# windingwind/seal-3d

Measured on AMD Instinct MI355X. Metric: train samples/s (NGP -O step on synthetic Lego 800x800 rays), higher is better.
Workload: dtype f16; 1 GPU; configs[1]: nerf_synthetic/lego-shaped NGP -O (hashgrid L16 F2 T2^19 + ffmlp 64x2/64x3 + raymarching), 800x800 cameras, 4096 rays/step/GPU; num_rays_per_gpu=4096, parallelism=ray-sharded dp1, pretrain_steps=384, launch=hip-graph replay

## Files before the change

### include/seal3d_hip.h

```cpp
#ifndef SEAL3D_HIP_H
#define SEAL3D_HIP_H

#include <stddef.h>
#include <stdint.h>

#ifdef __cplusplus
extern "C" {
#endif

typedef void* s3d_stream_t;

enum { S3D_F32 = 0, S3D_F16 = 1 };
enum { S3D_OK = 0, S3D_ERR_INVALID = 1, S3D_ERR_HIP = 2, S3D_ERR_UNSUPPORTED = 3 };

const char* s3d_last_error(void);
const char* s3d_version(void);


int s3d_near_far_from_aabb(const float* rays_o, const float* rays_d, const float* aabb, uint32_t N,
                           float min_near, float* nears, float* fars, float* noises, const int32_t* noise_step,
                           uint32_t noise_key, s3d_stream_t stream);

int s3d_sph_from_ray(const float* rays_o, const float* rays_d, float radius, uint32_t N, float* coords,
                     s3d_stream_t stream);
// ... 3 lines not shown

int s3d_morton3D(const int32_t* coords, uint32_t N, int32_t* indices, s3d_stream_t stream);

int s3d_morton3D_invert(const int32_t* indices, uint32_t N, int32_t* coords, s3d_stream_t stream);

int s3d_packbits(const float* grid, uint32_t N, float density_thresh, uint8_t* bitfield,
                 s3d_stream_t stream);

int s3d_sweep_draw(const double* u_uniform, const double* u_occupied, const int32_t* occ_csum, uint32_t N, uint32_t H,
                   float bound, float half_cell, uint32_t noise_key, const int32_t* noise_step, int32_t* cells,
                   float* xyzs, s3d_stream_t stream);
size_t s3d_sweep_update_workspace_size(uint32_t n_cells);
int s3d_sweep_update(float* density_grid, uint32_t n_cells, const int32_t* cells, const void* sigma, int sigma_dtype,
                     uint32_t n, float density_scale, float decay, void* workspace, size_t workspace_bytes,
                     float* grid_sum, int32_t* step_counter, s3d_stream_t stream);

size_t s3d_march_rays_train_workspace_size(uint32_t N, uint32_t max_steps);
int s3d_march_rays_train(const float* rays_o, const float* rays_d, const uint8_t* grid, float bound,
                         float dt_gamma, uint32_t max_steps, uint32_t N, uint32_t C, uint32_t H,
                         uint32_t M, const float* nears, const float* fars, float* xyzs, float* dirs,
                         float* deltas, int32_t* rays, int32_t* counter, const float* noises,
                         void* workspace, size_t workspace_bytes, int path, const float* aabb, float min_near,
                         const int32_t* noise_step, uint32_t noise_key, s3d_stream_t stream);

int s3d_composite_rays_train_forward(const float* sigmas, const float* rgbs, const float* deltas,
                                     const int32_t* rays, uint32_t M, uint32_t N, float T_thresh,
                                     float* weights_sum, float* depth, float* image, int path,
                                     s3d_stream_t stream);

int s3d_composite_rays_train_backward(const float* grad_weights_sum, const float* grad_image,
// ... 290 lines not shown
```

### seal-3d_amd/csrc/raymarching.hip

```cpp
#include "s3d_common.hpp"

namespace s3d {
namespace {

constexpr float kSqrt3 = 1.7320508075688772f;
constexpr float kRPi = 0.3183098861837907f;

__device__ __forceinline__ uint32_t expand_bits_any(uint32_t v) {
    v = (v * 0x00010001u) & 0xFF0000FFu;
    v = (v * 0x00000101u) & 0x0F00F00Fu;
    v = (v * 0x00000011u) & 0xC30C30C3u;
    v = (v * 0x00000005u) & 0x49249249u;
    return v;
}
__device__ __forceinline__ uint32_t expand_bits(uint32_t v) {
    v = (v | (v << 16)) & 0xFF0000FFu;
    v = (v | (v << 8)) & 0x0F00F00Fu;
    v = (v | (v << 4)) & 0xC30C30C3u;
    v = (v | (v << 2)) & 0x49249249u;
    return v;
}
__device__ __forceinline__ uint32_t morton3d(uint32_t x, uint32_t y, uint32_t z) {
    return expand_bits(x) | (expand_bits(y) << 1) | (expand_bits(z) << 2);
}
// ... 87 lines not shown
__global__ void k_morton3d(const int32_t* __restrict__ coords, uint32_t N, int32_t* __restrict__ indices) {
    for (uint32_t n = blockIdx.x * blockDim.x + threadIdx.x; n < N; n += gridDim.x * blockDim.x)
        indices[n] = (int32_t)(expand_bits_any((uint32_t)coords[n * 3]) | (expand_bits_any((uint32_t)coords[n * 3 + 1]) << 1) |
                               (expand_bits_any((uint32_t)coords[n * 3 + 2]) << 2));
}

__global__ void k_morton3d_invert(const int32_t* __restrict__ indices, uint32_t N, int32_t* __restrict__ coords) {
    for (uint32_t n = blockIdx.x * blockDim.x + threadIdx.x; n < N; n += gridDim.x * blockDim.x) {
        const int32_t ind = indices[n];
        coords[n * 3] = (int32_t)morton3d_invert((uint32_t)(ind >> 0));
        coords[n * 3 + 1] = (int32_t)morton3d_invert((uint32_t)(ind >> 1));
        coords[n * 3 + 2] = (int32_t)morton3d_invert((uint32_t)(ind >> 2));
    }
}

__global__ void k_packbits(const float* __restrict__ grid, uint32_t N, float thresh, uint8_t* __restrict__ bitfield) {
    const float4* g4 = reinterpret_cast<const float4*>(grid);
    for (uint32_t n = blockIdx.x * blockDim.x + threadIdx.x; n < N; n += gridDim.x * blockDim.x) {
        const float4 a = g4[n * 2], b = g4[n * 2 + 1];
        uint32_t bits = 0;
        bits |= (a.x > thresh) ? 1u : 0u;   bits |= (a.y > thresh) ? 2u : 0u;
        bits |= (a.z > thresh) ? 4u : 0u;   bits |= (a.w > thresh) ? 8u : 0u;
        bits |= (b.x > thresh) ? 16u : 0u;  bits |= (b.y > thresh) ? 32u : 0u;
        bits |= (b.z > thresh) ? 64u : 0u;  bits |= (b.w > thresh) ? 128u : 0u;
        bitfield[n] = (uint8_t)bits;
    }
}

__global__ void __launch_bounds__(256) k_sweep_draw(const double* __restrict__ u_uniform, const double* __restrict__ u_occupied,
                                                    const int32_t* __restrict__ occ_csum, uint32_t N, uint32_t H, float bound,
                                                    float half_cell, uint32_t noise_key, const int32_t* __restrict__ noise_step,
                                                    int32_t* __restrict__ cells, float* __restrict__ xyzs) {
    const uint32_t i = blockIdx.x * 256 + threadIdx.x;
    if (i >= 2 * N) return;
    const uint32_t H3 = H * H * H;
    uint32_t cell;
    if (i < N) {
        const double v = u_uniform[i] * (double)H3;
        cell = v >= (double)(H3 - 1) ? H3 - 1 : (uint32_t)v;
    } else {
        const int32_t total = occ_csum[H3 - 1];
        const int32_t pick = (int32_t)(u_occupied[i - N] * (double)total);
        uint32_t lo = 0, hi = H3;
        while (lo < hi) {
            const uint32_t mid = (lo + hi) >> 1;
            if (occ_csum[mid] > pick) hi = mid; else lo = mid + 1;
        }
        cell = lo < H3 ? lo : H3 - 1;
    }
    cells[i] = (int32_t)cell;
    const uint32_t step = noise_step ? (uint32_t)*noise_step : 0u;
    const float inv = 2.0f / (float)(H - 1), span = bound - half_cell;
#pragma unroll
    for (uint32_t d = 0; d < 3; d++) {
        const float c = (float)morton3d_invert(cell >> d);
        const float r = ray_noise(noise_key, step, 3u * i + d);
        xyzs[(size_t)i * 3 + d] = __builtin_fmaf(__builtin_fmaf(2.0f, r, -1.0f), half_cell, (c * inv - 1.0f) * span);
    }
}

__global__ void __launch_bounds__(256) k_sweep_fill(float* __restrict__ tmp, uint32_t n) {
    const uint32_t i = blockIdx.x * 256 + threadIdx.x;
    if (i < n) tmp[i] = -1.0f;
}
template <typename T>
__global__ void __launch_bounds__(256) k_sweep_scatter(const int32_t* __restrict__ cells, const T* __restrict__ sigma, uint32_t n,
                                                       float scale, float* __restrict__ tmp) {
    const uint32_t i = blockIdx.x * 256 + threadIdx.x;
    if (i >= n) return;
    const float v = (float)sigma[i] * scale;
    atomicMax(reinterpret_cast<int32_t*>(tmp) + cells[i], __float_as_int(v));
}
__global__ void __launch_bounds__(256) k_sweep_update(float* __restrict__ grid, const float* __restrict__ tmp, uint32_t n, float decay,
                                                      float* __restrict__ partial) {
    __shared__ float wsum[4];
    float acc = 0.0f;
    for (uint32_t i = blockIdx.x * 256 + threadIdx.x; i < n; i += gridDim.x * 256) {
        float g = grid[i];
        const float t = tmp[i];
        if (g >= 0.0f && t >= 0.0f) { g = fmaxf(g * decay, t); grid[i] = g; }
        acc += g > 0.0f ? g : 0.0f;
    }
#pragma unroll
    for (int d = 32; d >= 1; d >>= 1) acc += __shfl_xor(acc, d, 64);
    if ((threadIdx.x & 63) == 0) wsum[threadIdx.x >> 6] = acc;
    __syncthreads();
    if (threadIdx.x == 0) partial[blockIdx.x] = (wsum[0] + wsum[1]) + (wsum[2] + wsum[3]);
}
__global__ void __launch_bounds__(256) k_sweep_mean(const float* __restrict__ partial, uint32_t nblocks, float inv_n, float* __restrict__ mean,
                                                    int32_t* __restrict__ step_counter) {
    __shared__ float wsum[4];
    float acc = 0.0f;
    for (uint32_t i = threadIdx.x; i < nblocks; i += 256) acc += partial[i];
#pragma unroll
    for (int d = 32; d >= 1; d >>= 1) acc += __shfl_xor(acc, d, 64);
    if ((threadIdx.x & 63) == 0) wsum[threadIdx.x >> 6] = acc;
    __syncthreads();
    if (threadIdx.x == 0) {
        *mean = ((wsum[0] + wsum[1]) + (wsum[2] + wsum[3])) * inv_n;
        if (step_counter) *step_counter += 1;
    }
}

struct Ray {
    float ox, oy, oz, dx, dy, dz, rdx, rdy, rdz;
};
struct MarchParams {
    float bound, dt_gamma, dt_min, dt_max, rH, H3, Cf, Hf, Hm1, halfH;
    const uint8_t* grid;
};

__device__ __forceinline__ MarchParams make_params(float bound, float dt_gamma, uint32_t max_steps, uint32_t C,
                                                   uint32_t H, const uint8_t* grid) {
    MarchParams p;
    p.bound = bound; p.dt_gamma = dt_gamma;
// ... 1374 lines not shown

S3D_EXPORT int s3d_compact_alive(const int32_t* in, uint32_t n, int32_t* out, int32_t* n_out, void* workspace,
                                 size_t workspace_bytes, const int32_t* n_in_dev, s3d_stream_t stream) {
    S3D_REQUIRE(n_out, "compact_alive: null n_out");
    if (n == 0) { S3D_HIP(hipMemsetAsync(n_out, 0, sizeof(int32_t), as_stream(stream))); return S3D_OK; }
    S3D_REQUIRE(in && out && workspace && workspace_bytes >= s3d_compact_alive_workspace_size(n),
                "compact_alive: bad arguments");
    const uint32_t nw = div_up<uint32_t>(n, 64);
    hipLaunchKernelGGL(k_compact_count, dim3(nw), dim3(64), 0, as_stream(stream), in, n, (uint32_t*)workspace, n_in_dev);
    hipLaunchKernelGGL(k_compact_write, dim3(nw), dim3(64), 0, as_stream(stream), in, n, out, n_out,
                       (const uint32_t*)workspace, n_in_dev);
    return check_launch("compact_alive");
}

constexpr uint32_t kSweepBlocks = 1024;

S3D_EXPORT int s3d_sweep_draw(const double* u_uniform, const double* u_occupied, const int32_t* occ_csum, uint32_t N, uint32_t H,
                              float bound, float half_cell, uint32_t noise_key, const int32_t* noise_step, int32_t* cells,
                              float* xyzs, s3d_stream_t stream) {
    if (N == 0) return S3D_OK;
    S3D_REQUIRE(u_uniform && u_occupied && occ_csum && cells && xyzs, "sweep_draw: null pointer");
    S3D_REQUIRE(H >= 2 && H <= 1024 && (uint64_t)2 * N < (1ull << 31), "sweep_draw: unsupported grid size H=%u or N=%u", H, N);
    hipLaunchKernelGGL(k_sweep_draw, dim3(div_up<uint32_t>(2 * N, 256)), dim3(256), 0, as_stream(stream), u_uniform, u_occupied,
                       occ_csum, N, H, bound, half_cell, noise_key, noise_step, cells, xyzs);
    return check_launch("sweep_draw");
}

S3D_EXPORT size_t s3d_sweep_update_workspace_size(uint32_t n_cells) { return ((size_t)n_cells + kSweepBlocks) * sizeof(float); }

S3D_EXPORT int s3d_sweep_update(float* density_grid, uint32_t n_cells, const int32_t* cells, const void* sigma, int sigma_dtype,
                                uint32_t n, float density_scale, float decay, void* workspace, size_t workspace_bytes,
                                float* grid_sum, int32_t* step_counter, s3d_stream_t stream) {
    S3D_REQUIRE(density_grid && n_cells > 0 && (n == 0 || (cells && sigma)) && grid_sum, "sweep_update: null pointer");
    S3D_REQUIRE(sigma_dtype == S3D_F32 || sigma_dtype == S3D_F16, "sweep_update: sigma dtype must be f32 or f16");
    S3D_REQUIRE(workspace && workspace_bytes >= s3d_sweep_update_workspace_size(n_cells), "sweep_update: workspace too small");
    hipStream_t st = as_stream(stream);
    float* tmp = (float*)workspace;
    float* partial = tmp + n_cells;
    hipLaunchKernelGGL(k_sweep_fill, dim3(div_up<uint32_t>(n_cells, 256)), dim3(256), 0, st, tmp, n_cells);
    if (n) {
        if (sigma_dtype == S3D_F16)
            hipLaunchKernelGGL(k_sweep_scatter<_Float16>, dim3(div_up<uint32_t>(n, 256)), dim3(256), 0, st, cells, (const _Float16*)sigma, n,
                               density_scale, tmp);
        else
            hipLaunchKernelGGL(k_sweep_scatter<float>, dim3(div_up<uint32_t>(n, 256)), dim3(256), 0, st, cells, (const float*)sigma, n,
                               density_scale, tmp);
    }
    const uint32_t blocks = std::min<uint32_t>(kSweepBlocks, div_up<uint32_t>(n_cells, 256));
    hipLaunchKernelGGL(k_sweep_update, dim3(blocks), dim3(256), 0, st, density_grid, (const float*)tmp, n_cells, decay, partial);
    hipLaunchKernelGGL(k_sweep_mean, dim3(1), dim3(256), 0, st, (const float*)partial, blocks, 1.0f, grid_sum, step_counter);
    return check_launch("sweep_update");
}
```

### seal-3d_amd/nerf/renderer.py

```python
import math

import numpy as np
import torch
import torch.nn as nn

import raymarching
import s3d_hip


import contextlib

_null_context = contextlib.nullcontext


def _meshgrid(*args):
    return torch.meshgrid(*args, indexing="ij")


def sample_pdf(bins, weights, n_samples, det=False):
    weights = weights + 1e-5
    pdf = weights / torch.sum(weights, -1, keepdim=True)
    cdf = torch.cumsum(pdf, -1)
    cdf = torch.cat([torch.zeros_like(cdf[..., :1]), cdf], -1)
    if det:
# ... 3 lines not shown
        u = torch.rand(list(cdf.shape[:-1]) + [n_samples]).to(weights.device)
    u = u.contiguous()
    inds = torch.searchsorted(cdf, u, right=True)
    below = torch.clamp(inds - 1, min=0)
    above = torch.clamp(inds, max=cdf.shape[-1] - 1)
    pick = torch.stack([below, above], -1)
    shape = [pick.shape[0], pick.shape[1], cdf.shape[-1]]
    cdf_g = torch.gather(cdf.unsqueeze(1).expand(shape), 2, pick)
    bins_g = torch.gather(bins.unsqueeze(1).expand(shape), 2, pick)
    denom = cdf_g[..., 1] - cdf_g[..., 0]
    denom = torch.where(denom < 1e-5, torch.ones_like(denom), denom)
    t = (u - cdf_g[..., 0]) / denom
    return bins_g[..., 0] + t * (bins_g[..., 1] - bins_g[..., 0])


class NeRFRenderer(nn.Module):
    def __init__(self, bound=1, cuda_ray=False, density_scale=1, min_near=0.2, density_thresh=0.01, bg_radius=-1,
                 device_compaction=True, infer_batch_scale=1):
        super().__init__()
        self.bound = bound
        self.cascade = 1 + math.ceil(math.log2(bound))
        self.grid_size = 128
        self.density_scale = density_scale
        self.min_near = min_near
        self.density_thresh = density_thresh
        self.bg_radius = bg_radius
        self.device_compaction = device_compaction
        self.sync_every = 4
        self.infer_batch_scale = infer_batch_scale

        aabb = torch.FloatTensor([-bound, -bound, -bound, bound, bound, bound])
# ... 299 lines not shown

    @torch.no_grad()
    def _pick_occupied(self, cas, N):
        grid = self.density_grid[cas]
        csum = torch.cumsum(grid > 0, dim=0, dtype=torch.int32)
        pick = (self._sorted_uniform(N, grid.device) * csum[-1]).to(torch.int32)
        return torch.searchsorted(csum, pick, right=True).clamp_(max=grid.shape[0] - 1)

    @torch.no_grad()
    def partial_grid_update_device(self, decay=0.95):
        dev = self.density_grid.device
        H3 = self.grid_size ** 3
        N = H3 // 4
        if dev.type == "cuda" and self.density_grid.dtype == torch.float32:
            R = s3d_hip.RaymarchingBackend
            if getattr(self, "_sweep_step", None) is None or self._sweep_step.device != dev:
                self._sweep_step = torch.zeros(1, dtype=torch.int32, device=dev)
                self._sweep_key = torch.initial_seed() & 0xFFFFFFFF
            total = None
            for cas in range(self.cascade):
                bound, hgs = self._cascade_geometry(cas)
                grid = self.density_grid[cas]
                csum = torch.cumsum(grid > 0, dim=0, dtype=torch.int32)
                cells, xyzs = R.sweep_draw(self._sorted_uniform(N, dev), self._sorted_uniform(N, dev), csum, self.grid_size, bound,
                                           hgs, self._sweep_key + cas, self._sweep_step)
                sigma = self.density(xyzs)["sigma"].reshape(-1).detach()
                if sigma.dtype not in (torch.float16, torch.float32):
                    sigma = sigma.float()
                part = R.sweep_update(grid, cells, sigma.contiguous(), self.density_scale, decay,
                                      self._sweep_step if cas == self.cascade - 1 else None)
                total = part if total is None else total + part
            return total / self.density_grid.numel()
        tmp_grid = torch.full_like(self.density_grid, -1)
        for cas in range(self.cascade):
            indices = (self._sorted_uniform(N, dev) * H3).long().clamp_(max=H3 - 1)
            coords = raymarching.morton3D_invert(indices)
            occ = self._pick_occupied(cas, N)
            occ_coords = raymarching.morton3D_invert(occ)
            indices = torch.cat([indices, occ], dim=0)
            coords = torch.cat([coords, occ_coords], dim=0)
            tmp_grid[cas, indices] = self._query_cells(coords, cas).to(tmp_grid.dtype)
        valid = (self.density_grid >= 0) & (tmp_grid >= 0)
        self.density_grid.copy_(torch.where(valid, torch.maximum(self.density_grid * decay, tmp_grid), self.density_grid))
        g = self.density_grid.clamp(min=0)
        return g.view(-1, 4096).sum(dim=1).sum() / g.numel()

    @torch.no_grad()
    def finish_extra_state(self, mean_density_dev):
        total_step = min(16, self.local_step)
        counted = self.step_counter[:max(total_step, 1), 0].sum().float()
        mean_density, count_sum = torch.stack([mean_density_dev.float().reshape(()), counted]).tolist()
        self.mean_density = mean_density
        self.iter_density += 1
        thresh = min(self.mean_density, self.density_thresh)
        self.density_bitfield = raymarching.packbits(self.density_grid, thresh, self.density_bitfield)
        if total_step > 0:
            self.mean_count = int(count_sum / total_step)
        self.local_step = 0

    def run(self, rays_o, rays_d, num_steps=128, upsample_steps=128, bg_color=None, perturb=False, **kwargs):
        prefix = rays_o.shape[:-1]
        rays_o = rays_o.contiguous().view(-1, 3)
        rays_d = rays_d.contiguous().view(-1, 3)
# ... 67 lines not shown
```

### seal-3d_amd/nerf/trainer.py

```python
import math

import torch
import torch.nn.functional as F

from gridencoder.grid import bump_weights_epoch


def psnr(pred, target):
    return -10 * math.log10(float(torch.mean((pred.float() - target.float()) ** 2)) + 1e-20)


class _BgMse(torch.autograd.Function):

    @staticmethod
    def forward(ctx, image, weights_sum, gt, bg, expected_grad=None, depth=None, gt_depth=None, depth_weight=1.0):
        import s3d_hip
        image, weights_sum, gt = image.float().contiguous(), weights_sum.float().contiguous(), gt.float().contiguous()
        loss = torch.empty((), dtype=torch.float32, device=image.device)
        ctx.pre = None
        extra = {}
        if depth is not None:
            extra = dict(depth=depth.detach().float().contiguous().reshape(-1), gt_depth=gt_depth.float().contiguous().reshape(-1),
                         depth_weight=float(depth_weight))
        if expected_grad is not None and expected_grad.dtype == torch.float32 and expected_grad.numel() == 1:
# ... 271 lines not shown
        super().__init__(model, capturable=True, **kw)
        self.capture_collectives = capture_collectives
        self.collectives_in_graph = False
        dev = next(model.parameters()).device
        self.s_ro = torch.zeros(num_rays, 3, device=dev)
        self.s_rd = torch.zeros(num_rays, 3, device=dev)
        self.s_gt = torch.zeros(num_rays, 3, device=dev)
        self.s_bg = torch.ones(num_rays, 3, device=dev)
        self.budget_factor = budget_factor
        self.graph_extra_state = graph_extra_state
        self.ues_graph, self.ues_mean, self.ues_warm = None, None, False
        self.graph = None
        self.graph_opt = None
        self.n_captures = 0
        self.budget = 0
        self.s_loss = None
        self.s_counter = torch.zeros(2, dtype=torch.int32, device=dev)
        self.loss_ring = torch.zeros(1024, dtype=torch.float32, device=dev)
        self._pushes = 0
        self.s_cursor = torch.zeros(2, dtype=torch.int32, device=dev)
        self.noise_key = (torch.initial_seed() * 0x9E3779B1 + (self.dist.rank if self.dist is not None else 0) * 0x85EBCA6B) & 0xFFFFFFFF
        self._counter_ring = None
        self._ring_args = None
        self.s_index = torch.zeros(1, dtype=torch.int64, device=dev)
        self.s_inds_coarse = torch.zeros(1, num_rays, dtype=torch.int64, device=dev)
        self._graph_em = None
        self._graph_bg = False

    def static_batch(self):
        n = self.s_ro.shape[0]
# ... 82 lines not shown
            self.graph_opt = torch.cuda.CUDAGraph()
            with torch.cuda.graph(self.graph_opt, pool=self.graph.pool(), capture_error_mode=_CAPTURE_MODE):
                self._body_opt()
            self.collectives_in_graph = False
        model.step_counter = ring
        model._counter_prezeroed = False
        model._noise_step = None
        model.mean_count, model.local_step = saved

    def load_checkpoint(self, checkpoint, model_only=False):
        out = super().load_checkpoint(checkpoint, model_only=model_only)
        self._counter_ring = None
        self.graph = self.graph_opt = None
        return out

    def _maybe_update_extra_state(self):
        from .renderer import NeRFRenderer
        model = self.model
        if not (model.cuda_ray and self.global_step % self.update_extra_interval == 0):
            return False
        epilogue = getattr(model, "after_extra_state", None) if getattr(type(model), "extra_state_epilogue_only", False) else None
        plain = type(model).update_extra_state is NeRFRenderer.update_extra_state or epilogue is not None
        if not (self.graph_extra_state and plain and model.iter_density >= 16) or getattr(model, "dist_shard", None) is not None:
            return super()._maybe_update_extra_state()
        with torch.autocast("cuda", dtype=torch.float16, enabled=self.fp16):
            if self.ues_graph is None and not self.ues_warm:
                mean = model.partial_grid_update_device()
                self.ues_warm = True
            else:
                if self.ues_graph is None:
                    self.ues_graph = torch.cuda.CUDAGraph()
                    with torch.cuda.graph(self.ues_graph, capture_error_mode=_CAPTURE_MODE):
                        self.ues_mean = model.partial_grid_update_device()
                self.ues_graph.replay()
                mean = self.ues_mean
            model.finish_extra_state(mean)
            if epilogue is not None:
                epilogue()
        if self.dist is not None:
            self.dist.sync_extra_state(model)
        return True

    def _stage_inputs(self, rays_o, rays_d, gt_rgb, bg=None):
        dst, src = [self.s_ro, self.s_rd, self.s_gt], [rays_o, rays_d, gt_rgb]
        if bg is not None:
            dst.append(self.s_bg)
            src.append(bg)
        if all(a.data_ptr() == b.data_ptr() for a, b in zip(dst, src)):
# ... 24 lines not shown
            self._pushes += 1
        return slot

    def train_step(self, rays_o, rays_d, gt_rgb, bg_color=1, index=None, inds_coarse=None):
        self._em_batch = self._error_map_batch(index, inds_coarse, gt_rgb)
        try:
            return self._graphed_step(rays_o, rays_d, gt_rgb, bg_color)
        finally:
            self._em_batch = None

    def _graphed_step(self, rays_o, rays_d, gt_rgb, bg_color):
        model = self.model
        model.train()
        if self._maybe_update_extra_state():
            self.s_cursor[0].zero_()
            if self.graph is not None and (model.mean_count * 1.1 > self.budget or model.mean_count * 2 < self.budget):
                self.graph = None
        self.global_step += 1
        if self.graph is None and model.mean_count <= 0:
            loss = self._eager_step(rays_o, rays_d, gt_rgb, bg_color)
            self._sched_step()
            return loss
        per_ray = torch.is_tensor(bg_color)
        if per_ray:
            if type(self)._static_loss is not GraphedTrainer._static_loss:
                raise ValueError("GraphedTrainer: this trainer's captured criterion composites on bg_color=1")
            if not (bg_color.is_cuda and bg_color.dtype == torch.float32 and bg_color.numel() == self.s_bg.numel()):
                raise ValueError("GraphedTrainer: a per-ray background is an fp32 device tensor [num_rays, 3]")
            self._stage_inputs(rays_o, rays_d, gt_rgb, bg_color.detach())
        elif bg_color != 1:
            raise ValueError("GraphedTrainer: the captured step composites on the white background (bg_color=1) of the "
                             "BASELINE configs or on a per-ray background tensor; use Trainer for other background colours")
# ... 31 lines not shown
```

### seal-3d_amd/s3d_hip/__init__.py

```python
import ctypes as C
import os
import subprocess
import weakref

import torch

_HERE = os.path.dirname(os.path.abspath(__file__))
LIB_PATH = os.environ.get("S3D_HIP_LIB") or os.path.join(_HERE, "libseal3d_hip.so")
CSRC = os.path.join(os.path.dirname(_HERE), "csrc")

F32, F16 = 0, 1

EXPORTS = [
    "s3d_last_error", "s3d_version",
    "s3d_near_far_from_aabb", "s3d_sph_from_ray", "s3d_morton3D", "s3d_morton3D_invert", "s3d_mip_levels", "s3d_packbits",
    "s3d_march_rays_train_workspace_size", "s3d_march_rays_train",
    "s3d_sweep_draw", "s3d_sweep_update_workspace_size", "s3d_sweep_update",
    "s3d_composite_rays_train_forward", "s3d_composite_rays_train_backward", "s3d_composite_rays_train_loss",
    "s3d_march_rays", "s3d_composite_rays", "s3d_compact_alive_workspace_size", "s3d_compact_alive",
    "s3d_grid_level_scales", "s3d_grid_encode_forward", "s3d_grid_encode_forward_pair", "s3d_grid_corner_indices", "s3d_grid_encode_backward",
    "s3d_grid_encode_backward_workspace_size", "s3d_grid_encode_backward_control_size",
    "s3d_grad_total_variation",
    "s3d_sh_encode_forward", "s3d_sh_encode_backward", "s3d_freq_encode_forward", "s3d_freq_encode_backward", "s3d_freq_encode_pack_forward", "s3d_freq_encode_pack_backward",
    "s3d_ffmlp_forward", "s3d_ffmlp_inference", "s3d_ffmlp_ngp_pair_inference", "s3d_ffmlp_wgrad_reduce_pair", "s3d_ffmlp_backward_workspace_size", "s3d_ffmlp_backward",
    "s3d_ffmlp_fused_backward_supported",
    "s3d_ffmlp_allocate_splitk", "s3d_ffmlp_free_splitk",
    "s3d_grads_nonfinite", "s3d_adam_step", "s3d_adam_step_multi", "s3d_adam_advance", "s3d_scaler_update", "s3d_step_ring_push", "s3d_step_epilogue",
    "s3d_ngp_mid_forward", "s3d_ngp_mid_backward", "s3d_ngp_mid2_forward", "s3d_ngp_mid2_backward", "s3d_ngp_rgb_forward", "s3d_ngp_rgb_backward",
    "s3d_bg_mse_forward", "s3d_bg_mse_backward", "s3d_bg_targets", "s3d_l1_pair_workspace_size", "s3d_l1_pair_loss",
    "s3d_seal_bbox_map", "s3d_seal_map_color", "s3d_seal_map_color_image", "s3d_seal_brush_map", "s3d_seal_anchor_map", "s3d_grid_encode_backward_adam", "s3d_vm_features_forward",
    "s3d_aabb_normalize", "s3d_weighted_abs_sum_workspace_size", "s3d_weighted_abs_sum", "s3d_pack_linear_chain", "s3d_unpack_linear_chain",
    "s3d_vm_backward_max_bins", "s3d_vm_backward_keys", "s3d_vm_backward_bins_workspace_size", "s3d_vm_backward_bins",
# ... 18 lines not shown


def lib():
    global _lib
    if _lib is None:
        if not os.path.exists(LIB_PATH):
            raise RuntimeError(
                f"seal3d HIP extension not built: {LIB_PATH} is missing. Run `python -c 'import __graft_entry__ as g; "
                "g.build()'` (needs hipcc). There is no CPU fallback for the product path.")
        l = C.CDLL(LIB_PATH)
        l.s3d_last_error.restype = C.c_char_p
        l.s3d_version.restype = C.c_char_p
        for name in ("s3d_march_rays_train_workspace_size", "s3d_compact_alive_workspace_size",
                     "s3d_ffmlp_backward_workspace_size", "s3d_grid_encode_backward_workspace_size",
                     "s3d_grid_encode_backward_control_size", "s3d_l1_pair_workspace_size",
                     "s3d_sweep_update_workspace_size", "s3d_vm_backward_bins_workspace_size", "s3d_vm_backward_stage_bytes",
                     "s3d_weighted_abs_sum_workspace_size", "s3d_background_backward_workspace_size",
                     "s3d_vm_background_backward_workspace_size"):
            getattr(l, name).restype = C.c_size_t
        l.s3d_vm_backward_max_bins.restype = C.c_uint32
        l.s3d_grid_level_scales.restype = None
        _lib = l
    return _lib


def _check(rc, what):
    if rc != 0:
        msg = lib().s3d_last_error().decode("utf-8", "replace")
        raise RuntimeError(f"{what} failed (code {rc}): {msg}")


# ... 191 lines not shown

    @staticmethod
    def sweep_update(density_grid, cells, sigma, density_scale, decay, step_counter=None):
        _need(density_grid, torch.float32, "density_grid"); _need(cells, torch.int32, "cells")
        if sigma.dtype not in (torch.float16, torch.float32) or sigma.numel() != cells.numel():
            raise RuntimeError("sweep_update: sigma must be fp16 / fp32, one per cell sample")
        if step_counter is not None:
            _need(step_counter, torch.int32, "step_counter")
        n_cells = density_grid.numel()
        ws = _ws.get(lib().s3d_sweep_update_workspace_size(_u(n_cells)), density_grid.device)
        out = torch.empty((), dtype=torch.float32, device=density_grid.device)
        _check(lib().s3d_sweep_update(_p(density_grid), _u(n_cells), _p(cells), _p(sigma), C.c_int(_dt(sigma)), _u(cells.numel()),
                                      _f(density_scale), _f(decay), _p(ws), C.c_size_t(ws.numel()), _p(out), _p(step_counter),
                                      _stream()), "sweep_update")
        return out

    @staticmethod
    def sph_from_ray(rays_o, rays_d, radius, N, coords):
        _need(rays_o, torch.float32, "rays_o")
        _check(lib().s3d_sph_from_ray(_p(rays_o), _p(rays_d), _f(radius), _u(N), _p(coords), _stream()),
               "sph_from_ray")

    @staticmethod
    def morton3D(coords, N, indices):
        _need(coords, torch.int32, "coords")
        _check(lib().s3d_morton3D(_p(coords), _u(N), _p(indices), _stream()), "morton3D")

    @staticmethod
    def morton3D_invert(indices, N, coords):
        _need(indices, torch.int32, "indices")
# ... 1092 lines not shown
```

Before: 647.7 million samples/s.

## Move density-grid sweep draw, update and threshold record fully onto device kernels

Adds native GPU kernels for the occupancy-grid sweep. Occupied-cell sampling now uses per-block bit masks plus a scanned count array instead of a full cumsum, scatter and update are fused per cascade, and a tail kernel computes the mean, threshold and step count into a device record that packbits reads directly. The trainer defers the graph budget check while extra-state work is pending, so the host does not have to sync to read mean_count. This adds more kernels and a deferred budget check that may recapture graphs one step late.

```diff
diff --git a/include/seal3d_hip.h b/include/seal3d_hip.h
--- a/include/seal3d_hip.h
+++ b/include/seal3d_hip.h
@@ -41,6 +41,18 @@
 int s3d_sweep_update(float* density_grid, uint32_t n_cells, const int32_t* cells, const void* sigma, int sigma_dtype,
                      uint32_t n, float density_scale, float decay, void* workspace, size_t workspace_bytes,
                      float* grid_sum, int32_t* step_counter, s3d_stream_t stream);
+
+size_t s3d_sweep_draw_native_workspace_size(uint32_t H);
+int s3d_sweep_draw_native(const double* u_uniform, const double* u_occupied, const float* density_grid, uint32_t N, uint32_t H,
+                          float bound, float half_cell, uint32_t noise_key, const int32_t* noise_step, float* tmp, int32_t* cells,
+                          float* xyzs, void* workspace, size_t workspace_bytes, s3d_stream_t stream);
+uint32_t s3d_sweep_partial_stride(void);
+int s3d_sweep_scatter_update(float* density_grid, uint32_t n_cells, const int32_t* cells, const void* sigma, int sigma_dtype,
+                             uint32_t sigma_stride, uint32_t n, float density_scale, float decay, float* tmp, float* partial,
+                             s3d_stream_t stream);
+int s3d_sweep_tail(const float* partial, uint32_t cascades, uint32_t n_cells, float density_thresh, const int32_t* step_ring,
+                   const int32_t* local_step, int32_t* sweep_step, void* record, s3d_stream_t stream);
+int s3d_packbits_record(const float* grid, uint32_t N, const void* record, uint8_t* bitfield, s3d_stream_t stream);
 
 size_t s3d_march_rays_train_workspace_size(uint32_t N, uint32_t max_steps);
 int s3d_march_rays_train(const float* rays_o, const float* rays_d, const uint8_t* grid, float bound,
diff --git a/seal-3d_amd/csrc/raymarching.hip b/seal-3d_amd/csrc/raymarching.hip
--- a/seal-3d_amd/csrc/raymarching.hip
+++ b/seal-3d_amd/csrc/raymarching.hip
@@ -125,7 +125,7 @@
     }
 }
 
-__global__ void k_packbits(const float* __restrict__ grid, uint32_t N, float thresh, uint8_t* __restrict__ bitfield) {
+__device__ __forceinline__ void packbits_rows(const float* __restrict__ grid, uint32_t N, float thresh, uint8_t* __restrict__ bitfield) {
     const float4* g4 = reinterpret_cast<const float4*>(grid);
     for (uint32_t n = blockIdx.x * blockDim.x + threadIdx.x; n < N; n += gridDim.x * blockDim.x) {
         const float4 a = g4[n * 2], b = g4[n * 2 + 1];
@@ -137,7 +137,36 @@
         bitfield[n] = (uint8_t)bits;
     }
 }
-
+__global__ void k_packbits(const float* __restrict__ grid, uint32_t N, float thresh, uint8_t* __restrict__ bitfield) {
+    packbits_rows(grid, N, thresh, bitfield);
+}
+
+struct SweepRecord {
+    float mean;
+    float thresh;
+    uint32_t count_lo;
+    uint32_t count_hi;
+};
+__global__ void k_packbits_record(const float* __restrict__ grid, uint32_t N, const SweepRecord* __restrict__ record,
+                                  uint8_t* __restrict__ bitfield) {
+    packbits_rows(grid, N, record->thresh, bitfield);
+}
+
+__device__ __forceinline__ uint32_t sweep_uniform_cell(double u, uint32_t H3) {
+    const double v = u * (double)H3;
+    return v >= (double)(H3 - 1) ? H3 - 1 : (uint32_t)v;
+}
+__device__ __forceinline__ void sweep_emit(uint32_t i, uint32_t cell, uint32_t H, float bound, float half_cell, uint32_t noise_key,
+                                           uint32_t step, int32_t* __restrict__ cells, float* __restrict__ xyzs) {
+    cells[i] = (int32_t)cell;
+    const float inv = 2.0f / (float)(H - 1), span = bound - half_cell;
+#pragma unroll
+    for (uint32_t d = 0; d < 3; d++) {
+        const float c = (float)morton3d_invert(cell >> d);
+        const float r = ray_noise(noise_key, step, 3u * i + d);
+        xyzs[(size_t)i * 3 + d] = __builtin_fmaf(__builtin_fmaf(2.0f, r, -1.0f), half_cell, (c * inv - 1.0f) * span);
+    }
+}
 __global__ void __launch_bounds__(256) k_sweep_draw(const double* __restrict__ u_uniform, const double* __restrict__ u_occupied,
                                                     const int32_t* __restrict__ occ_csum, uint32_t N, uint32_t H, float bound,
                                                     float half_cell, uint32_t noise_key, const int32_t* __restrict__ noise_step,
@@ -147,8 +176,7 @@
     const uint32_t H3 = H * H * H;
     uint32_t cell;
     if (i < N) {
-        const double v = u_uniform[i] * (double)H3;
-        cell = v >= (double)(H3 - 1) ? H3 - 1 : (uint32_t)v;
+        cell = sweep_uniform_cell(u_uniform[i], H3);
     } else {
         const int32_t total = occ_csum[H3 - 1];
         const int32_t pick = (int32_t)(u_occupied[i - N] * (double)total);
@@ -159,14 +187,136 @@
         }
         cell = lo < H3 ? lo : H3 - 1;
     }
-    cells[i] = (int32_t)cell;
     const uint32_t step = noise_step ? (uint32_t)*noise_step : 0u;
-    const float inv = 2.0f / (float)(H - 1), span = bound - half_cell;
-#pragma unroll
-    for (uint32_t d = 0; d < 3; d++) {
-        const float c = (float)morton3d_invert(cell >> d);
-        const float r = ray_noise(noise_key, step, 3u * i + d);
-        xyzs[(size_t)i * 3 + d] = __builtin_fmaf(__builtin_fmaf(2.0f, r, -1.0f), half_cell, (c * inv - 1.0f) * span);
+    sweep_emit(i, cell, H, bound, half_cell, noise_key, step, cells, xyzs);
+}
+
+constexpr uint32_t kScanBlock = 1024;
+constexpr uint32_t kSweepCntLds = 4096;
+
+template <typename T>
+__device__ __forceinline__ T block_scan_exclusive(T mine, T* sh, T& total) {
+    const uint32_t lane = threadIdx.x & 63u, w = threadIdx.x >> 6;
+    T incl = mine;
+#pragma unroll
+    for (int d = 1; d < 64; d <<= 1) {
+        const T up = __shfl_up(incl, d, 64);
+        if (lane >= (uint32_t)d) incl = incl + up;
+    }
+    if (lane == 63u) sh[w] = incl;
+    __syncthreads();
+    const T w0 = sh[0], w1 = sh[1], w2 = sh[2], w3 = sh[3];
+    __syncthreads();
+    const T before = __shfl_up(incl, 1, 64);
+    const T lanes = lane == 0u ? T(0) : before;
+    total = ((w0 + w1) + w2) + w3;
+    const T off = w == 0 ? T(0) : (w == 1 ? w0 : (w == 2 ? w0 + w1 : (w0 + w1) + w2));
+    return off + lanes;
+}
+
+__global__ void __launch_bounds__(256) k_sweep_partials(const float* __restrict__ grid, uint32_t H3, float* __restrict__ tmp,
+                                                        int32_t* __restrict__ cnt, uint32_t* __restrict__ occ_bits, uint32_t nbc) {
+    __shared__ int32_t shi[4];
+    __shared__ uint32_t words[32];
+    const uint32_t t = threadIdx.x;
+    for (uint32_t b = blockIdx.x; b < nbc; b += gridDim.x) {
+        const uint32_t c0 = b * kScanBlock + 4u * t;
+        uint32_t nib = 0;
+#pragma unroll
+        for (uint32_t q = 0; q < 4; q++)
+            if (c0 + q < H3) {
+                nib |= grid[c0 + q] > 0.0f ? (1u << q) : 0u;
+                tmp[c0 + q] = -1.0f;
+            }
+        if (t < 32) words[t] = 0;
+        __syncthreads();
+        if (nib) atomicOr(&words[t >> 3], nib << (4u * (t & 7u)));
+        __syncthreads();
+        if (t < 32) occ_bits[b * 32u + t] = words[t];
+        int32_t total;
+        (void)block_scan_exclusive((int32_t)__popc(nib), shi, total);
+        if (t == 0) cnt[b] = total;
+    }
+}
+
+template <typename T>
+__device__ __forceinline__ void scan_inclusive_in_place(T* __restrict__ a, uint32_t n, T* sh) {
+    T carry = T(0);
+    for (uint32_t base = 0; base < n; base += kScanBlock) {
+        const uint32_t j0 = base + 4u * threadIdx.x;
+        T l[4], acc = T(0);
+#pragma unroll
+        for (uint32_t q = 0; q < 4; q++) {
+            const T v = (j0 + q < n) ? a[j0 + q] : T(0);
+            acc = q == 0 ? v : acc + v;
+            l[q] = acc;
+        }
+        T total;
+        const T pre = carry + block_scan_exclusive(acc, sh, total);
+#pragma unroll
+        for (uint32_t q = 0; q < 4; q++)
+            if (j0 + q < n) a[j0 + q] = pre + l[q];
+        carry = carry + total;
+    }
+}
+__global__ void __launch_bounds__(256) k_sweep_scan(int32_t* __restrict__ cnt, uint32_t nbc) {
+    __shared__ int32_t shi[4];
+    scan_inclusive_in_place(cnt, nbc, shi);
+}
+
+__device__ __forceinline__ uint32_t sweep_occupied_cell(int32_t pick, const int32_t* __restrict__ incl_cnt,
+                                                        const uint32_t* __restrict__ occ_bits, uint32_t nbc, uint32_t H3) {
+    uint32_t lo = 0, hi = nbc;
+    while (lo < hi) {
+        const uint32_t mid = (lo + hi) >> 1;
+        if (incl_cnt[mid] > pick) hi = mid; else lo = mid + 1;
+    }
+    if (lo >= nbc) return H3 - 1;
+    const int32_t r = pick - (lo ? incl_cnt[lo - 1] : 0);
+    const uint4* __restrict__ w4 = reinterpret_cast<const uint4*>(occ_bits + (size_t)lo * 32u);
+    uint4 v[8];
+#pragma unroll
+    for (int k = 0; k < 8; k++) v[k] = w4[k];
+    uint32_t word = 0, at = 32;
+    int32_t rest = 0, before = 0;
+#pragma unroll
+    for (int w = 0; w < 32; w++) {
+        const uint4 q = v[w >> 2];
+        const uint32_t x = (w & 3) == 0 ? q.x : ((w & 3) == 1 ? q.y : ((w & 3) == 2 ? q.z : q.w));
+        const int32_t c = (int32_t)__popc(x);
+        if (at == 32 && r < before + c) { at = (uint32_t)w; word = x; rest = r - before; }
+        before += c;
+    }
+    if (at == 32) return H3 - 1;
+    for (; rest > 0; rest--) word &= word - 1u;
+    const uint32_t cell = lo * kScanBlock + at * 32u + (uint32_t)(__ffs((int)word) - 1);
+    return cell < H3 ? cell : H3 - 1;
+}
+
+__global__ void __launch_bounds__(256) k_sweep_draw_native(const double* __restrict__ u_uniform, const double* __restrict__ u_occupied,
+                                                           const int32_t* __restrict__ incl_cnt, const uint32_t* __restrict__ occ_bits,
+                                                           uint32_t nbc, uint32_t N, uint32_t H, float bound, float half_cell,
+                                                           uint32_t noise_key, const int32_t* __restrict__ noise_step,
+                                                           int32_t* __restrict__ cells, float* __restrict__ xyzs) {
+    const uint32_t H3 = H * H * H;
+    const uint32_t step = noise_step ? (uint32_t)*noise_step : 0u;
+    __shared__ int32_t sh_cnt[kSweepCntLds];
+    const int32_t* cnt = incl_cnt;
+    if (nbc <= kSweepCntLds) {
+        for (uint32_t i = threadIdx.x; i < nbc; i += 256) sh_cnt[i] = incl_cnt[i];
+        __syncthreads();
+        cnt = sh_cnt;
+    }
+    const int32_t occupied = cnt[nbc - 1];
+    const uint32_t j0 = blockIdx.x * kScanBlock + 4u * threadIdx.x;
+#pragma unroll
+    for (uint32_t q = 0; q < 4; q++) {
+        const uint32_t j = j0 + q;
+        if (j < N) {
+            sweep_emit(j, sweep_uniform_cell(u_uniform[j], H3), H, bound, half_cell, noise_key, step, cells, xyzs);
+            const int32_t pick = (int32_t)(u_occupied[j] * (double)occupied);
+            sweep_emit(N + j, sweep_occupied_cell(pick, cnt, occ_bits, nbc, H3), H, bound, half_cell, noise_key, step, cells, xyzs);
+        }
     }
 }
 
@@ -175,11 +325,11 @@
     if (i < n) tmp[i] = -1.0f;
 }
 template <typename T>
-__global__ void __launch_bounds__(256) k_sweep_scatter(const int32_t* __restrict__ cells, const T* __restrict__ sigma, uint32_t n,
-                                                       float scale, float* __restrict__ tmp) {
+__global__ void __launch_bounds__(256) k_sweep_scatter(const int32_t* __restrict__ cells, const T* __restrict__ sigma, uint32_t stride,
+                                                       uint32_t n, float scale, float* __restrict__ tmp) {
     const uint32_t i = blockIdx.x * 256 + threadIdx.x;
     if (i >= n) return;
-    const float v = (float)sigma[i] * scale;
+    const float v = (float)sigma[(size_t)i * stride] * scale;
     atomicMax(reinterpret_cast<int32_t*>(tmp) + cells[i], __float_as_int(v));
 }
 __global__ void __launch_bounds__(256) k_sweep_update(float* __restrict__ grid, const float* __restrict__ tmp, uint32_t n, float decay,
@@ -198,18 +348,47 @@
     __syncthreads();
     if (threadIdx.x == 0) partial[blockIdx.x] = (wsum[0] + wsum[1]) + (wsum[2] + wsum[3]);
 }
+__device__ __forceinline__ float sweep_sum_partials(const float* __restrict__ partial, uint32_t nblocks, float* wsum) {
+    float acc = 0.0f;
+    for (uint32_t i = threadIdx.x; i < nblocks; i += 256) acc += partial[i];
+#pragma unroll
+    for (int d = 32; d >= 1; d >>= 1) acc += __shfl_xor(acc, d, 64);
+    if ((threadIdx.x & 63) == 0) wsum[threadIdx.x >> 6] = acc;
+    __syncthreads();
+    const float s = (wsum[0] + wsum[1]) + (wsum[2] + wsum[3]);
+    __syncthreads();
+    return s;
+}
 __global__ void __launch_bounds__(256) k_sweep_mean(const float* __restrict__ partial, uint32_t nblocks, float inv_n, float* __restrict__ mean,
                                                     int32_t* __restrict__ step_counter) {
     __shared__ float wsum[4];
-    float acc = 0.0f;
-    for (uint32_t i = threadIdx.x; i < nblocks; i += 256) acc += partial[i];
-#pragma unroll
-    for (int d = 32; d >= 1; d >>= 1) acc += __shfl_xor(acc, d, 64);
-    if ((threadIdx.x & 63) == 0) wsum[threadIdx.x >> 6] = acc;
-    __syncthreads();
+    const float s = sweep_sum_partials(partial, nblocks, wsum);
     if (threadIdx.x == 0) {
-        *mean = ((wsum[0] + wsum[1]) + (wsum[2] + wsum[3])) * inv_n;
+        *mean = s * inv_n;
         if (step_counter) *step_counter += 1;
+    }
+}
+__global__ void __launch_bounds__(256) k_sweep_tail(const float* __restrict__ partial, uint32_t cascades, uint32_t stride,
+                                                    uint32_t nblocks, float inv_n, float density_thresh,
+                                                    const int32_t* __restrict__ step_ring, const int32_t* __restrict__ local_step,
+                                                    int32_t* __restrict__ sweep_step, SweepRecord* __restrict__ record) {
+    __shared__ float wsum[4];
+    float total = 0.0f;
+    for (uint32_t c = 0; c < cascades; c++) {
+        const float s = sweep_sum_partials(partial + (size_t)c * stride, nblocks, wsum);
+        total = c == 0 ? s : total + s;
+    }
+    if (threadIdx.x == 0) {
+        const float mean = total * inv_n;
+        record->mean = mean;
+        record->thresh = density_thresh < mean ? density_thresh : mean;
+        int32_t rows = *local_step;
+        rows = rows < 0 ? 0 : (rows > 16 ? 16 : rows);
+        int64_t count = 0;
+        for (int32_t r = 0; r < rows; r++) count += step_ring[2 * r];
+        record->count_lo = (uint32_t)((uint64_t)count & 0xFFFFFFFFull);
+        record->count_hi = (uint32_t)((uint64_t)count >> 32);
+        if (sweep_step) *sweep_step += 1;
     }
 }
 
@@ -1614,6 +1793,17 @@
 }
 
 constexpr uint32_t kSweepBlocks = 1024;
+static uint32_t sweep_update_blocks(uint32_t n_cells) { return std::min<uint32_t>(kSweepBlocks, div_up<uint32_t>(n_cells, 256)); }
+static void launch_sweep_scatter(const int32_t* cells, const void* sigma, int sigma_dtype, uint32_t stride, uint32_t n, float scale,
+                                 float* tmp, hipStream_t st) {
+    if (n == 0) return;
+    if (sigma_dtype == S3D_F16)
+        hipLaunchKernelGGL(k_sweep_scatter<_Float16>, dim3(div_up<uint32_t>(n, 256)), dim3(256), 0, st, cells, (const _Float16*)sigma,
+                           stride, n, scale, tmp);
+    else
+        hipLaunchKernelGGL(k_sweep_scatter<float>, dim3(div_up<uint32_t>(n, 256)), dim3(256), 0, st, cells, (const float*)sigma, stride,
+                           n, scale, tmp);
+}
 
 S3D_EXPORT int s3d_sweep_draw(const double* u_uniform, const double* u_occupied, const int32_t* occ_csum, uint32_t N, uint32_t H,
                               float bound, float half_cell, uint32_t noise_key, const int32_t* noise_step, int32_t* cells,
@@ -1638,16 +1828,66 @@
     float* tmp = (float*)workspace;
     float* partial = tmp + n_cells;
     hipLaunchKernelGGL(k_sweep_fill, dim3(div_up<uint32_t>(n_cells, 256)), dim3(256), 0, st, tmp, n_cells);
-    if (n) {
-        if (sigma_dtype == S3D_F16)
-            hipLaunchKernelGGL(k_sweep_scatter<_Float16>, dim3(div_up<uint32_t>(n, 256)), dim3(256), 0, st, cells, (const _Float16*)sigma, n,
-                               density_scale, tmp);
-        else
-            hipLaunchKernelGGL(k_sweep_scatter<float>, dim3(div_up<uint32_t>(n, 256)), dim3(256), 0, st, cells, (const float*)sigma, n,
-                               density_scale, tmp);
-    }
-    const uint32_t blocks = std::min<uint32_t>(kSweepBlocks, div_up<uint32_t>(n_cells, 256));
+    launch_sweep_scatter(cells, sigma, sigma_dtype, 1, n, density_scale, tmp, st);
+    const uint32_t blocks = sweep_update_blocks(n_cells);
     hipLaunchKernelGGL(k_sweep_update, dim3(blocks), dim3(256), 0, st, density_grid, (const float*)tmp, n_cells, decay, partial);
     hipLaunchKernelGGL(k_sweep_mean, dim3(1), dim3(256), 0, st, (const float*)partial, blocks, 1.0f, grid_sum, step_counter);
     return check_launch("sweep_update");
 }
+
+static uint32_t sweep_cell_blocks(uint32_t H) { return div_up<uint32_t>(H * H * H, kScanBlock); }
+
+S3D_EXPORT size_t s3d_sweep_draw_native_workspace_size(uint32_t H) { return (size_t)sweep_cell_blocks(H) * 33 * sizeof(uint32_t); }
+
+S3D_EXPORT int s3d_sweep_draw_native(const double* u_uniform, const double* u_occupied, const float* density_grid, uint32_t N,
+                                     uint32_t H, float bound, float half_cell, uint32_t noise_key, const int32_t* noise_step,
+                                     float* tmp, int32_t* cells, float* xyzs, void* workspace, size_t workspace_bytes,
+                                     s3d_stream_t stream) {
+    S3D_REQUIRE(u_uniform && u_occupied && density_grid && tmp && cells && xyzs && N > 0, "sweep_draw_native: null pointer or N = 0");
+    S3D_REQUIRE(H >= 2 && H <= 1024 && (uint64_t)2 * N < (1ull << 31), "sweep_draw_native: unsupported grid size H=%u or N=%u", H, N);
+    S3D_REQUIRE(workspace && ((uintptr_t)workspace & 15) == 0 && workspace_bytes >= s3d_sweep_draw_native_workspace_size(H),
+                "sweep_draw_native: workspace too small or misaligned");
+    const uint32_t nbc = sweep_cell_blocks(H), H3 = H * H * H;
+    uint32_t* occ_bits = (uint32_t*)workspace;
+    int32_t* cnt = (int32_t*)(occ_bits + (size_t)nbc * 32);
+    hipStream_t st = as_stream(stream);
+    hipLaunchKernelGGL(k_sweep_partials, dim3(std::min<uint32_t>(nbc, 4096)), dim3(256), 0, st, density_grid, H3, tmp, cnt, occ_bits, nbc);
+    hipLaunchKernelGGL(k_sweep_scan, dim3(1), dim3(256), 0, st, cnt, nbc);
+    hipLaunchKernelGGL(k_sweep_draw_native, dim3(div_up<uint32_t>(N, kScanBlock)), dim3(256), 0, st, u_uniform, u_occupied,
+                       (const int32_t*)cnt, (const uint32_t*)occ_bits, nbc, N, H, bound, half_cell, noise_key, noise_step, cells, xyzs);
+    return check_launch("sweep_draw_native");
+}
+
+S3D_EXPORT uint32_t s3d_sweep_partial_stride(void) { return kSweepBlocks; }
+
+S3D_EXPORT int s3d_sweep_scatter_update(float* density_grid, uint32_t n_cells, const int32_t* cells, const void* sigma, int sigma_dtype,
+                                        uint32_t sigma_stride, uint32_t n, float density_scale, float decay, float* tmp,
+                                        float* partial, s3d_stream_t stream) {
+    S3D_REQUIRE(density_grid && n_cells > 0 && (n == 0 || (cells && sigma)) && tmp && partial, "sweep_scatter_update: null pointer");
+    S3D_REQUIRE(sigma_dtype == S3D_F32 || sigma_dtype == S3D_F16, "sweep_scatter_update: sigma dtype must be f32 or f16");
+    hipStream_t st = as_stream(stream);
+    launch_sweep_scatter(cells, sigma, sigma_dtype, sigma_stride, n, density_scale, tmp, st);
+    hipLaunchKernelGGL(k_sweep_update, dim3(sweep_update_blocks(n_cells)), dim3(256), 0, st, density_grid, (const float*)tmp, n_cells,
+                       decay, partial);
+    return check_launch("sweep_scatter_update");
+}
+
+S3D_EXPORT int s3d_sweep_tail(const float* partial, uint32_t cascades, uint32_t n_cells, float density_thresh,
+                              const int32_t* step_ring, const int32_t* local_step, int32_t* sweep_step, void* record,
+                              s3d_stream_t stream) {
+    S3D_REQUIRE(partial && cascades > 0 && n_cells > 0 && step_ring && local_step && record, "sweep_tail: null pointer");
+    S3D_REQUIRE(((uintptr_t)record & 3) == 0, "sweep_tail: record must be 4-byte aligned");
+    const float inv_n = 1.0f / (float)((uint64_t)cascades * n_cells);
+    hipLaunchKernelGGL(k_sweep_tail, dim3(1), dim3(256), 0, as_stream(stream), partial, cascades, kSweepBlocks,
+                       sweep_update_blocks(n_cells), inv_n, density_thresh, step_ring, local_step, sweep_step, (SweepRecord*)record);
+    return check_launch("sweep_tail");
+}
+
+S3D_EXPORT int s3d_packbits_record(const float* grid, uint32_t N, const void* record, uint8_t* bitfield, s3d_stream_t stream) {
+    if (N == 0) return S3D_OK;
+    S3D_REQUIRE(grid && bitfield && record, "packbits_record: null pointer");
+    S3D_REQUIRE(((uintptr_t)grid & 15) == 0 && ((uintptr_t)record & 3) == 0, "packbits_record: grid must be 16-byte aligned");
+    hipLaunchKernelGGL(k_packbits_record, dim3(stream_grid(N, 256)), dim3(256), 0, as_stream(stream), grid, N,
+                       (const SweepRecord*)record, bitfield);
+    return check_launch("packbits_record");
+}
diff --git a/seal-3d_amd/nerf/renderer.py b/seal-3d_amd/nerf/renderer.py
--- a/seal-3d_amd/nerf/renderer.py
+++ b/seal-3d_amd/nerf/renderer.py
@@ -41,7 +41,69 @@
     return bins_g[..., 0] + t * (bins_g[..., 1] - bins_g[..., 0])
 
 
+class _SweepState:
+
+    def __init__(self, dev):
+        self.device = dev
+        self.step = torch.zeros(1, dtype=torch.int32, device=dev)
+        self.local_step = torch.zeros(1, dtype=torch.int32, device=dev)
+        self.record = torch.zeros(4, dtype=torch.int32, device=dev)
+        self.host = torch.zeros(4, dtype=torch.int32).pin_memory()
+        self.event = torch.cuda.Event()
+        self.key = torch.initial_seed() & 0xFFFFFFFF
+        self.pending = None
+
+    def __deepcopy__(self, memo):
+        return None
+
+    def __reduce__(self):
+        return (type(None), ())
+
+
 class NeRFRenderer(nn.Module):
+    _mean_density = 0
+    _mean_count = 0
+    _sweep = None
+
+    @property
+    def mean_density(self):
+        self._resolve_extra_state()
+        return self._mean_density
+
+    @mean_density.setter
+    def mean_density(self, value):
+        self._resolve_extra_state()
+        self._mean_density = value
+
+    @property
+    def mean_count(self):
+        self._resolve_extra_state()
+        return self._mean_count
+
+    @mean_count.setter
+    def mean_count(self, value):
+        self._resolve_extra_state()
+        self._mean_count = value
+
+    def __getstate__(self):
+        self._resolve_extra_state()
+        return self.__dict__
+
+    def extra_state_pending(self):
+        return self._sweep is not None and self._sweep.pending is not None
+
+    def _resolve_extra_state(self):
+        st = self._sweep
+        if st is None or st.pending is None:
+            return
+        total_step, st.pending = st.pending, None
+        st.event.synchronize()
+        rec = st.host.numpy()
+        self._mean_density = float(rec.view(np.float32)[0])
+        if total_step > 0:
+            count = int(rec.view(np.uint32)[2]) | (int(rec.view(np.uint32)[3]) << 32)
+            self._mean_count = int(count / total_step)
+
     def __init__(self, bound=1, cuda_ray=False, density_scale=1, min_near=0.2, density_thresh=0.01, bg_radius=-1,
                  device_compaction=True, infer_batch_scale=1):
         super().__init__()
@@ -371,23 +433,25 @@
         N = H3 // 4
         if dev.type == "cuda" and self.density_grid.dtype == torch.float32:
             R = s3d_hip.RaymarchingBackend
-            if getattr(self, "_sweep_step", None) is None or self._sweep_step.device != dev:
-                self._sweep_step = torch.zeros(1, dtype=torch.int32, device=dev)
-                self._sweep_key = torch.initial_seed() & 0xFFFFFFFF
-            total = None
+            st = self._sweep
+            if st is None or st.device != dev:
+                st = self._sweep = _SweepState(dev)
+            if not torch.cuda.is_current_stream_capturing():
+                self.stage_extra_state()
+            tmp = torch.empty(H3, dtype=torch.float32, device=dev)
+            partial = torch.empty(self.cascade, R.sweep_partial_stride(), dtype=torch.float32, device=dev)
             for cas in range(self.cascade):
                 bound, hgs = self._cascade_geometry(cas)
                 grid = self.density_grid[cas]
-                csum = torch.cumsum(grid > 0, dim=0, dtype=torch.int32)
-                cells, xyzs = R.sweep_draw(self._sorted_uniform(N, dev), self._sorted_uniform(N, dev), csum, self.grid_size, bound,
-                                           hgs, self._sweep_key + cas, self._sweep_step)
+                cells, xyzs = R.sweep_draw_native(self._sorted_uniform(N, dev), self._sorted_uniform(N, dev), grid, self.grid_size,
+                                                  bound, hgs, tmp, st.key + cas, st.step)
                 sigma = self.density(xyzs)["sigma"].reshape(-1).detach()
                 if sigma.dtype not in (torch.float16, torch.float32):
                     sigma = sigma.float()
-                part = R.sweep_update(grid, cells, sigma.contiguous(), self.density_scale, decay,
-                                      self._sweep_step if cas == self.cascade - 1 else None)
-                total = part if total is None else total + part
-            return total / self.density_grid.numel()
+                R.sweep_scatter_update(grid, cells, sigma, self.density_scale, decay, tmp, partial[cas])
+            R.sweep_tail(partial, H3, self.density_thresh, self.step_counter, st.local_step, st.step, st.record)
+            R.packbits_record(self.density_grid, self.cascade * H3 // 8, st.record, self.density_bitfield)
+            return st.record
         tmp_grid = torch.full_like(self.density_grid, -1)
         for cas in range(self.cascade):
             indices = (self._sorted_uniform(N, dev) * H3).long().clamp_(max=H3 - 1)
@@ -403,7 +467,21 @@
         return g.view(-1, 4096).sum(dim=1).sum() / g.numel()
 
     @torch.no_grad()
+    def stage_extra_state(self):
+        if self._sweep is not None:
+            self._sweep.local_step.fill_(int(self.local_step))
+
+    @torch.no_grad()
     def finish_extra_state(self, mean_density_dev):
+        st = self._sweep
+        if st is not None and mean_density_dev is st.record:
+            self._resolve_extra_state()
+            st.host.copy_(st.record, non_blocking=True)
+            st.event.record()
+            st.pending = min(16, self.local_step)
+            self.iter_density += 1
+            self.local_step = 0
+            return
         total_step = min(16, self.local_step)
         counted = self.step_counter[:max(total_step, 1), 0].sum().float()
         mean_density, count_sum = torch.stack([mean_density_dev.float().reshape(()), counted]).tolist()
diff --git a/seal-3d_amd/nerf/trainer.py b/seal-3d_amd/nerf/trainer.py
--- a/seal-3d_amd/nerf/trainer.py
+++ b/seal-3d_amd/nerf/trainer.py
@@ -309,6 +309,7 @@
         self.graph_opt = None
         self.n_captures = 0
         self.budget = 0
+        self._budget_check_due = False
         self.s_loss = None
         self.s_counter = torch.zeros(2, dtype=torch.int32, device=dev)
         self.loss_ring = torch.zeros(1024, dtype=torch.float32, device=dev)
@@ -421,6 +422,11 @@
         self.graph = self.graph_opt = None
         return out
 
+    def _check_budget(self):
+        mean = self.model.mean_count
+        if self.graph is not None and (mean * 1.1 > self.budget or mean * 2 < self.budget):
+            self.graph = None
+
     def _maybe_update_extra_state(self):
         from .renderer import NeRFRenderer
         model = self.model
@@ -430,6 +436,9 @@
         plain = type(model).update_extra_state is NeRFRenderer.update_extra_state or epilogue is not None
         if not (self.graph_extra_state and plain and model.iter_density >= 16) or getattr(model, "dist_shard", None) is not None:
             return super()._maybe_update_extra_state()
+        if self._budget_check_due:
+            self._budget_check_due = False
+            self._check_budget()
         with torch.autocast("cuda", dtype=torch.float16, enabled=self.fp16):
             if self.ues_graph is None and not self.ues_warm:
                 mean = model.partial_grid_update_device()
@@ -439,6 +448,7 @@
                     self.ues_graph = torch.cuda.CUDAGraph()
                     with torch.cuda.graph(self.ues_graph, capture_error_mode=_CAPTURE_MODE):
                         self.ues_mean = model.partial_grid_update_device()
+                model.stage_extra_state()
                 self.ues_graph.replay()
                 mean = self.ues_mean
             model.finish_extra_state(mean)
@@ -493,8 +503,11 @@
         model.train()
         if self._maybe_update_extra_state():
             self.s_cursor[0].zero_()
-            if self.graph is not None and (model.mean_count * 1.1 > self.budget or model.mean_count * 2 < self.budget):
-                self.graph = None
+            pending = getattr(model, "extra_state_pending", None)
+            if pending is not None and pending():
+                self._budget_check_due = True
+            else:
+                self._check_budget()
         self.global_step += 1
         if self.graph is None and model.mean_count <= 0:
             loss = self._eager_step(rays_o, rays_d, gt_rgb, bg_color)
diff --git a/seal-3d_amd/s3d_hip/__init__.py b/seal-3d_amd/s3d_hip/__init__.py
--- a/seal-3d_amd/s3d_hip/__init__.py
+++ b/seal-3d_amd/s3d_hip/__init__.py
@@ -16,6 +16,8 @@
     "s3d_near_far_from_aabb", "s3d_sph_from_ray", "s3d_morton3D", "s3d_morton3D_invert", "s3d_mip_levels", "s3d_packbits",
     "s3d_march_rays_train_workspace_size", "s3d_march_rays_train",
     "s3d_sweep_draw", "s3d_sweep_update_workspace_size", "s3d_sweep_update",
+    "s3d_sweep_draw_native_workspace_size", "s3d_sweep_draw_native", "s3d_sweep_partial_stride", "s3d_sweep_scatter_update",
+    "s3d_sweep_tail", "s3d_packbits_record",
     "s3d_composite_rays_train_forward", "s3d_composite_rays_train_backward", "s3d_composite_rays_train_loss",
     "s3d_march_rays", "s3d_composite_rays", "s3d_compact_alive_workspace_size", "s3d_compact_alive",
     "s3d_grid_level_scales", "s3d_grid_encode_forward", "s3d_grid_encode_forward_pair", "s3d_grid_corner_indices", "s3d_grid_encode_backward",
@@ -64,7 +66,7 @@
         for name in ("s3d_march_rays_train_workspace_size", "s3d_compact_alive_workspace_size",
                      "s3d_ffmlp_backward_workspace_size", "s3d_grid_encode_backward_workspace_size",
                      "s3d_grid_encode_backward_control_size", "s3d_l1_pair_workspace_size",
-                     "s3d_sweep_update_workspace_size", "s3d_vm_backward_bins_workspace_size", "s3d_vm_backward_stage_bytes",
+                     "s3d_sweep_update_workspace_size", "s3d_sweep_draw_native_workspace_size", "s3d_vm_backward_bins_workspace_size", "s3d_vm_backward_stage_bytes",
                      "s3d_weighted_abs_sum_workspace_size", "s3d_background_backward_workspace_size",
                      "s3d_vm_background_backward_workspace_size"):
             getattr(l, name).restype = C.c_size_t
@@ -286,6 +288,62 @@
                                       _f(density_scale), _f(decay), _p(ws), C.c_size_t(ws.numel()), _p(out), _p(step_counter),
                                       _stream()), "sweep_update")
         return out
+
+    @staticmethod
+    def sweep_draw_native(u_uniform, u_occupied, density_grid, H, bound, half_cell, tmp, noise_key=0, noise_step=None):
+        _need(u_uniform, torch.float64, "u_uniform"); _need(u_occupied, torch.float64, "u_occupied")
+        _need(density_grid, torch.float32, "density_grid"); _need(tmp, torch.float32, "tmp")
+        H3, dev = int(H) ** 3, density_grid.device
+        N = u_uniform.numel()
+        if u_occupied.numel() != N or density_grid.numel() != H3 or tmp.numel() != H3:
+            raise RuntimeError("sweep_draw_native: u_uniform / u_occupied are [N], density_grid and tmp [H^3]")
+        if noise_step is not None:
+            _need(noise_step, torch.int32, "noise_step")
+        ws = _ws.get(lib().s3d_sweep_draw_native_workspace_size(_u(H)), dev)
+        cells = torch.empty(2 * N, dtype=torch.int32, device=dev)
+        xyzs = torch.empty(2 * N, 3, dtype=torch.float32, device=dev)
+        _check(lib().s3d_sweep_draw_native(_p(u_uniform), _p(u_occupied), _p(density_grid), _u(N), _u(H), _f(bound), _f(half_cell),
+                                           _u(int(noise_key) & 0xFFFFFFFF), _p(noise_step), _p(tmp), _p(cells), _p(xyzs), _p(ws),
+                                           C.c_size_t(ws.numel()), _stream()), "sweep_draw_native")
+        return cells, xyzs
+
+    @staticmethod
+    def sweep_partial_stride():
+        return int(lib().s3d_sweep_partial_stride())
+
+    @staticmethod
+    def sweep_scatter_update(density_grid, cells, sigma, density_scale, decay, tmp, partial):
+        _need(density_grid, torch.float32, "density_grid"); _need(cells, torch.int32, "cells")
+        _need(tmp, torch.float32, "tmp"); _need(partial, torch.float32, "partial")
+        if sigma.dtype not in (torch.float16, torch.float32) or sigma.dim() != 1 or sigma.numel() != cells.numel() or not sigma.is_cuda:
+            raise RuntimeError("sweep_scatter_update: sigma must be a 1-D fp16 / fp32 GPU tensor, one per cell sample")
+        if tmp.numel() != density_grid.numel() or partial.numel() < RaymarchingBackend.sweep_partial_stride():
+            raise RuntimeError("sweep_scatter_update: tmp is [n_cells], partial [sweep_partial_stride()]")
+        stride = sigma.stride(0) if sigma.numel() > 1 else 1
+        if stride < 1:
+            raise RuntimeError("sweep_scatter_update: sigma must have a positive stride")
+        _check(lib().s3d_sweep_scatter_update(_p(density_grid), _u(density_grid.numel()), _p(cells), C.c_void_p(sigma.data_ptr()),
+                                              C.c_int(_dt(sigma)), _u(stride), _u(cells.numel()), _f(density_scale), _f(decay),
+                                              _p(tmp), _p(partial), _stream()), "sweep_scatter_update")
+
+    @staticmethod
+    def sweep_tail(partial, n_cells, density_thresh, step_ring, local_step, sweep_step, record):
+        _need(partial, torch.float32, "partial"); _need(step_ring, torch.int32, "step_ring")
+        _need(local_step, torch.int32, "local_step"); _need(record, torch.int32, "record")
+        if partial.dim() != 2 or partial.shape[1] != RaymarchingBackend.sweep_partial_stride() or step_ring.shape != (16, 2) \
+                or record.numel() != 4:
+            raise RuntimeError("sweep_tail: partial is [cascades, sweep_partial_stride()], step_ring [16, 2], record int32 [4]")
+        if sweep_step is not None:
+            _need(sweep_step, torch.int32, "sweep_step")
+        _check(lib().s3d_sweep_tail(_p(partial), _u(partial.shape[0]), _u(n_cells), _f(density_thresh), _p(step_ring),
+                                    _p(local_step), _p(sweep_step), _p(record), _stream()), "sweep_tail")
+
+    @staticmethod
+    def packbits_record(grid, N, record, bitfield):
+        _need(grid, torch.float32, "grid"); _need(record, torch.int32, "record"); _need(bitfield, torch.uint8, "bitfield")
+        if grid.numel() != 8 * int(N) or bitfield.numel() < int(N) or record.numel() != 4:
+            raise RuntimeError("packbits_record: grid holds 8 N cells, bitfield N bytes, record int32 [4]")
+        _check(lib().s3d_packbits_record(_p(grid), _u(N), _p(record), _p(bitfield), _stream()), "packbits_record")
 
     @staticmethod
     def sph_from_ray(rays_o, rays_d, radius, N, coords):
```

Measured after the change: 663.4 million samples/s (median of 6 runs). 2.4% higher.
